# michaelwillett/GPU-ICP-SLAM

Measured on AMD Instinct MI355X. Metric: particle-scan evals/sec (1081 beams x N particles), full particleFilter step, KD path, higher is better.
Workload: dtype f32; 1 GPU; synthetic 1081-beam scans, 100000 particles/GPU, 100000-point KD map, full SLAM step (disperse+score+weights+ICP/SVD+map update+resample); particles_global=100000, parallelism=particles sharded x1, map replicated, kd_size_end=191383

## Files before the change

### gpu-icp-slam_amd/build.py

```python
import fcntl
import hashlib
import os
import shutil
import subprocess

HERE = os.path.dirname(os.path.abspath(__file__))
CSRC = os.path.join(HERE, "csrc")
OBJ = os.path.join(HERE, "build")
LIB = os.path.join(HERE, "libpfslam_hip.so")
INC = os.path.join("..", "..", "include", "pfslam.h")
UNITS = {
    "pfslam_hip.hip": ["pf_math.h", "kd_device.h", "kd_cells.hip.inc", "pfslam_stages.hip.inc", "pfslam_frame.hip.inc", "pfslam_register.hip.inc", "pfslam_register_batch.hip.inc", "pfslam_search.hip.inc", "pfslam_search_scan.hip.inc", "pfslam_search_cov.hip.inc", "pfslam_search_wide.hip.inc", "pfslam_search_best.hip.inc", INC],
    "kd_host.cpp": [INC],
}
FLAGS = ["--offload-arch=gfx950", "-O3", "-std=c++17", "-ffp-contract=off", "-fPIC",
         "-Wall", "-Wno-unused-function", "-Wno-unused-result"] + os.environ.get("PFSLAM_EXTRA_FLAGS", "").split()


def hipcc():
    for c in (os.environ.get("HIPCC"), "/opt/rocm/bin/hipcc", shutil.which("hipcc")):
        if c and os.path.exists(c):
            return c
    raise RuntimeError("hipcc not found: libpfslam_hip.so cannot be built (there is no CPU fallback)")


def _digest(files):
    h = hashlib.sha1(" ".join(FLAGS).encode())
    for f in files:
        with open(os.path.join(CSRC, f), "rb") as fh:
            h.update(f.encode() + b"\0" + fh.read())
    return h.hexdigest()


def _unit_digest(src, deps):
    return _digest([src] + deps)


def _read(path):
    try:
        with open(path) as fh:
            return fh.read().strip()
    except OSError:
        return ""


# ... 40 lines not shown
```

### gpu-icp-slam_amd/csrc/kd_cells.hip.inc

```

#define PF_CELL_SUB 2
#define PF_CELL_WIN (2560 * PF_CELL_SUB)
#define PF_CELL_LIST_CAP (1 << 19)
#define PF_CELL_POOL_CAP (1 << 22)
#define PF_CELL_MAXC 12
#define PF_CELL_RUN 32
#define PF_CELL_MAXR 14
#define PF_CELL_MARK_MAX 4096
#define PF_CELL_PENDING 0xFFFFFFFFu
#define PF_CELL_FALLBACK 0xFFFFFFFEu
enum { PF_CS_COUNT = 0, PF_CS_POOL, PF_CS_SNAP, PF_CS_PAD3, PF_CS_LIST_CAP, PF_CS_POOL_CAP, PF_CS_FLAGS, PF_CS_PAD, PF_CS_ROWS, PF_CS_N1, PF_CS_N2,
       PF_CS_NONE, PF_CS_CUR_FRESH, PF_CS_CUR_EXT, PF_CS_CUR_REUSED, PF_CS_CUR_CLAIMED, PF_CS_WORDS = 32,
       PF_CS_OX = 128, PF_CS_OY = 129, PF_CS_ALLOC = 256 };
#define PF_CF_LIST_FULL 1
#define PF_CF_POOL_FULL 2
#define PF_CF_NEED_ORIGIN 4
#define PF_CF_FAR 8
#define PF_CELL_DRIFT_MAX 120
#define PF_REC_WORDS 96
#define PF_REC_TERM 4
#define PF_REC_CAND 20
#define PF_REC_PAR 36
#define PF_REC_RC 52
#define PF_REC_POOL 76
// ... 783 lines not shown
#undef S_CY
#undef S_PP
#undef S_PC
#undef S_CT
#undef S_PI
#undef S_R
#undef S_RX
#undef S_RY
__device__ __forceinline__ float cell_dist2(const uint4 cd, float wx, float wy)
{
    typedef float f32x2 __attribute__((ext_vector_type(2)));
    const f32x2 nxy = {__uint_as_float(cd.x), __uint_as_float(cd.y)};
    const f32x2 pxy = {wx, wy};
    const f32x2 d = nxy - pxy;
    const f32x2 dd = d * d;
    return dd.x + dd.y;
}
__device__ __forceinline__ bool cell_visit(const uint4 cd, float wx, float wy, float &sBest)
{
    const float s = cell_dist2(cd, wx, wy);
    const float sGuard = sBest * PF_GUARD_K;
    bool take = s < sGuard;
    const bool inBand = (s < sBest) != take;
    if (__builtin_amdgcn_ballot_w64(inBand) != 0ull) {
        float sb = sBest;
        asm volatile("" : "+v"(sb));
        take = take | (inBand && pf::fsqrt(s) < pf::fsqrt(sb));
    }
    sBest = take ? s : sBest;
    return take;
}

#define PF_ROW_SLACK 4
template <bool CENSUS = false, int GUARD = 1>
__global__ __launch_bounds__(64) void k_score_kd_cells(const float *__restrict__ px, const float *__restrict__ py,
                                                       const float *__restrict__ pth, int n, const float *__restrict__ scan,
                                                       const pf::BeamParts *__restrict__ beams, int nb, int beams_per_chunk, pf::KdView tree,
                                                       CellGeom geo, const unsigned *__restrict__ tab, const uint4 *__restrict__ pool,
                                                       const int *__restrict__ cs, const int *__restrict__ order, int direct,
                                                       float *__restrict__ out, int out_mode, pf::KdCensus *__restrict__ census = nullptr,
                                                       unsigned long long *__restrict__ probe = nullptr, const double2 *__restrict__ tparts = nullptr)
{
    pf_stamp(probe);
    const int g = blockIdx.x, slot = g * 64 + threadIdx.x;
    const int j0 = blockIdx.y * beams_per_chunk;
    const int j1 = min(nb, j0 + beams_per_chunk);
    const bool real = slot < n;
    const int i = order ? order[min(slot, n - 1)] : min(slot, n - 1);
    const float x = px[i], y = py[i], th = pth[i];
    pf::AngleParts T;
    if (tparts) {
        const double2 tp = tparts[i];
        T.c = tp.x;
        T.s = tp.y;
        T.a = (double)th;
    } else T = pf::angle_parts(th);
    const int ox = cs[PF_CS_OX], oy = cs[PF_CS_OY];
    const float inv2x = 2.0f * geo.invx, inv2y = 2.0f * geo.invy;
    const pf::kd_rsrc_t tab_rsrc = pf::kd_rsrc(tab), pool_rsrc = pf::kd_rsrc(pool);
    float acc = 0.0f, wpend = 0.0f;
    pf::KdCensusLocal cl = {0, 0, 0, 0, 0, 0, 0, 0};
    auto stage_a = [&](int j, float &wx, float &wy, unsigned &e) -> bool {
        const float r = scan[j];
        if (!(fabsf(r) < PF_RANGE_NEVER)) return false;
        beam_end_point<GUARD>(beams, j, r, th, T, wx, wy);
        if (!(fabsf(wx) < PF_LIDAR_RANGE && fabsf(wy) < PF_LIDAR_RANGE)) return false;
        wx += x;
        wy += y;
        e = 0u;
        float gx, gy;
        int cx = sub_index_fast(wx, inv2x, gx), cy = sub_index_fast(wy, inv2y, gy);
        const float g = fminf(gx, gy);
        bool ok = g > 0.0f;
        if (__builtin_amdgcn_fcmpf(g, 0.0f, 2 ) != __builtin_amdgcn_ballot_w64(true)) {
            if (!ok && fabsf(wx) < 1e6f && fabsf(wy) < 1e6f) {
                cx = sub_index(wx, geo.resx, geo.invx);
                cy = sub_index(wy, geo.resy, geo.invy);
                float lox, loy, hi, cell_lo;
                sub_edges(cx, geo.resx, lox, hi, cell_lo);
// ... 83 lines not shown
#pragma unroll
                    for (int q = 0; q < 4; q++)
                        if (k0 + q < n1) {
                            const bool take = cell_visit(cd[q], wx, wy, sBest);
                            pk = take ? cd[q].z : pk;
                            pcoord = take ? __uint_as_float(cd[q].w) : pcoord;
                        }
                }
                b = (int)(pk & 0x3fffffffu);
                if (pk < 0xC0000000u && n2 != 0) {
                    float hd = (pk < 0x40000000u ? wx : wy) - pcoord;
                    hd = (int)pk < 0 ? 0.0f : hd;
                    const float h2 = hd * hd;
                    bool pass = h2 < sBest * PF_GUARD_K;
                    const bool inBand = (!pass && h2 * PF_GUARD_K <= sBest) || sBest < 1e-30f;
                    if (__builtin_amdgcn_ballot_w64(inBand) != 0ull) {
                        float sb = sBest;
                        asm volatile("" : "+v"(sb));
                        pass = inBand ? fabsf(hd) < pf::fsqrt(sb) : pass;
                    }
                    if (pass) b = resolve(wx, wy, sBest, b, off + n1, n2);
                }
            }
            acc += wpend;
            wpend = tree.w[b];
        }
        cok = nok; cwx = nwx; cwy = nwy; ce = ne;
    }
    acc += wpend;
    if (CENSUS) pf::census_flush(cl, census);
    if (real && out_mode == 0) out[(size_t)blockIdx.y * n + (direct ? i : slot)] = acc;
    if (real && out_mode == 3) ((short *)out)[(size_t)blockIdx.y * n + slot] = (short)(int)acc;
    if (out_mode == 4) ((short *)out)[((size_t)g * gridDim.y + blockIdx.y) * 64 + threadIdx.x] = real ? (short)(int)acc : (short)0;
}
```

### gpu-icp-slam_amd/csrc/pfslam_frame.hip.inc

```

#define PF_FRAME_RING 4
enum { PF_FS_BOUND = 0, PF_FS_WALKED = 4, PF_FS_TICKET = 8, PF_FS_ICP = 9, PF_FS_WORDS = 16 };
enum { PF_WC_WALLS = 0, PF_WC_NEW, PF_WC_FLAGS, PF_WC_SIZE, PF_WC_WORDS = 4 };

enum { PF_FL_REDUCED = 0, PF_FL_TREE, PF_FL_ORDER, PF_FL_ICP, PF_FL_SCAN, PF_FL_FTAIL, PF_FL_POSEG , PF_FL_WORDS = 8 };
__device__ __forceinline__ void flag_store(int *word, int ticket) { __hip_atomic_store(word, ticket, __ATOMIC_RELEASE, __HIP_MEMORY_SCOPE_AGENT); }
__device__ __forceinline__ bool flag_wait(const int *word, int ticket, int *err)
{
    const unsigned long long t0 = wall_clock64(), limit = g_gate_ticks;
    while (__hip_atomic_load(word, __ATOMIC_ACQUIRE, __HIP_MEMORY_SCOPE_AGENT) - ticket < 0) {
        __builtin_amdgcn_s_sleep(8);
        if (wall_clock64() - t0 > limit) {
            if (err) __hip_atomic_store(err, ticket, __ATOMIC_RELAXED, __HIP_MEMORY_SCOPE_SYSTEM);
            return false;
        }
    }
    return true;
}
__global__ void k_gate(const int *__restrict__ word, int ticket, int *__restrict__ err)
{
    if (threadIdx.x == 0) flag_wait(word, ticket, err);
}
__global__ void k_gate_signal(int *__restrict__ done_word, int done_ticket, const int *__restrict__ word, int ticket, int *__restrict__ err)
{
// ... 908 lines not shown
    CHK(dalloc(&h->cloud, 8));
    HIPCHK(hipMemsetAsync(h->cloud, 0, 32, h->stream));
    CHK(dalloc(&h->sigr, (size_t)PF_FRAME_RING * 80));
    HIPCHK(hipMemsetAsync(h->sigr, 0, (size_t)PF_FRAME_RING * 80 * 4, h->stream));
    CHK(dalloc(&h->order_ring, (size_t)PF_FRAME_RING * h->n));
    hipEvent_t *evs[] = {&h->ev_reduced, &h->ev_tree2, &h->ev_order, &h->ev_icp, &h->ev_ftail, &h->ev_shift, &h->ev_poseg,
                         &h->ev_marked_r[0], &h->ev_marked_r[1], &h->ev_marked_r[2], &h->ev_marked_r[3],
                         &h->ev_walked_r[0], &h->ev_walked_r[1], &h->ev_walked_r[2], &h->ev_walked_r[3],
                         &h->ev_tail[0], &h->ev_tail[1], &h->ev_tail[2]};
    for (hipEvent_t *e : evs) HIPCHK(pf_event_create(e, hipEventDisableTiming));
    return 0;
}
static int gates_decide(pfslam_handle *h, bool *use)
{
    if (h->gates && !h->gates_tested) {
        if (h->pipe_live) CHK(settle_staged(h));
        hipStream_t st[4] = {h->stream, h->aux, h->fstream, h->cstream};
        for (hipStream_t q : st) HIPCHK(hipStreamSynchronize(q));
        bool ok = false;
        CHK(gates_selftest(h, &ok));
        h->gates_ok = ok;
        h->gates_tested = true;
        if (!ok && getenv("PFSLAM_VERBOSE")) fprintf(stderr, "pfslam: streams share a hardware queue: the frame's cross-stream edges stay events\n");
    }
    const bool want = h->gates && h->gates_ok && g_live_handles.load() == 1;
    if (h->pipe_live && want != h->gates_live) CHK(settle_staged(h));
    h->gates_live = want;
    *use = want;
    return 0;
}

static void frame_free(pfslam_handle *h)
{
    void *bufs[] = {h->fs, h->wcounts, h->flags, h->order_tmp, h->tparts, h->wall_c2, h->wall_xy2, h->wall_leaf2, h->wall_new2, h->wall_runs, h->wall_keys_s, h->wall_c2s, h->fstats, h->cloud, h->sigr, h->order_ring, h->pgroup, h->probe};
    for (void *b : bufs)
        if (b) (void)hipFree(b);
    hipEvent_t evs[] = {h->ev_reduced, h->ev_tree2, h->ev_order, h->ev_icp, h->ev_ftail, h->ev_shift, h->ev_poseg,
                        h->ev_marked_r[0], h->ev_marked_r[1], h->ev_marked_r[2], h->ev_marked_r[3],
                        h->ev_walked_r[0], h->ev_walked_r[1], h->ev_walked_r[2], h->ev_walked_r[3], h->ev_tail[0], h->ev_tail[1], h->ev_tail[2]};
    for (hipEvent_t e : evs)
        if (e) (void)hipEventDestroy(e);
    if (h->gate_err) (void)hipHostFree(h->gate_err);
}

static int join_all(pfslam_handle *h)
{
    if (!h->pipe_live || h->serial) return 0;
    hipStream_t tails[3] = {h->aux, h->fstream, h->cstream};
    for (int k = 0; k < 3; k++) {
        HIPCHK(hipEventRecord(h->ev_tail[k], tails[k]));
        HIPCHK(hipStreamWaitEvent(h->stream, h->ev_tail[k], 0));
    }
    return 0;
}

static bool frame_v2_ok(pfslam_handle *h, int *chunks_out, int *bpc_out)
{
    if (h->timing >= 2 || h->kd_size <= 0 || !h->integral_w || h->nb > 4096) return false;
    if (!org_use_cells(h, nullptr, true)) return false;
    const int chunks = score_chunks(h);
    const int bpc = (h->nb + chunks - 1) / chunks;
    const int used = (h->nb + bpc - 1) / bpc;
    if (used < 2 || !((float)bpc * h->w_absmax <= 32767.0f)) return false;
    if ((h->gn + PF_SCAN_TILE - 1) / PF_SCAN_TILE > 4096) return false;
    *chunks_out = used;
    *bpc_out = bpc;
    return true;
}

static int probe_slot_ptr(pfslam_handle *h, int id, unsigned long long **out)
{
    *out = (h->probe && h->probe_frames > 0) ? h->probe + (size_t)(h->cur_seq % h->probe_frames) * PF_PROBE_SLOTS + id : nullptr;
    return 0;
}
#define PB(id) (h->probe ? h->probe + (size_t)(seq % h->probe_frames) * PF_PROBE_SLOTS + (id) : (unsigned long long *)nullptr)

struct FvCtx {
    hipStream_t P, C, F, K;
    int seq, s4, s2, lag, groups, world;
    bool gates, serial, sync_cells, sharded, multi, ftail_gate;
    CellGeom geo;
    pf::KdView tv;
    long long *stats, *stats_next;
    float *sig, *sig_next, *icp_dbg;
    int *order, *fl;
    HostHeader *hdr;
    PoseSrc psrc;
};
static FvCtx fv_ctx(pfslam_handle *h)
{
    FvCtx c;
    const auto &fv = h->fv;
    c.serial = fv.serial;
    c.sync_cells = fv.sync_cells;
    c.sharded = fv.sharded;
// ... 50 lines not shown
    HIPCHK(hipEventRecord(h->ev_marked_r[s4], K));
    if (!c.sync_cells && h->pipe_live) FV_EDGE_WAIT(K, PF_FL_TREE, h->ev_tree2, 1);
    if (c.sync_cells) {
        h->cells_passes++;
        hipLaunchKernelGGL(k_cells_update<true>, dim3(PF_CELLS_GRID), dim3(64), 0, K, c.tv, c.geo, h->cell_tab, (const int *)h->cell_list, h->cell_state, h->cell_pool,
                           h->cell_rec, h->cells_gen, (const int *)nullptr, 0, 0, 0, CellPass{nullptr, nullptr, nullptr, nullptr, 0}, PB(PB_WALK));
        hipLaunchKernelGGL(k_fs_walked, dim3(1), dim3(64), 0, K, h->fs, (const int *)h->cell_state);
    } else {
        hipLaunchKernelGGL(k_cells_update<false>, dim3(PF_CELLS_WALK_GRID), dim3(64), 0, K, c.tv, c.geo, h->cell_tab, (const int *)h->cell_list, h->cell_state,
                           h->cell_pool, h->cell_rec, h->cells_gen, (const int *)nullptr, 0, 0, 0,
                           CellPass{h->fs + PF_FS_WALKED + ((seq - 1) & 3), h->fs + PF_FS_WALKED + s4, nullptr, h->fs + PF_FS_BOUND + s4, 0}, PB(PB_WALK));
    }
    HIPCHK(hipGetLastError());
    HIPCHK(hipEventRecord(h->ev_walked_r[s4], K));
    return 0;
}

static int frame_v2_begin(pfslam_handle *h, int frame, const float *scan_host, int used, int bpc, bool sharded)
{
    CHK(frame_alloc(h));
    if (!h->cell_tab) CHK(cells_alloc(h));
    const int groups = (h->n + 63) / 64;
    if (!h->group_box) CHK(dalloc(&h->group_box, (size_t)groups));
    if (!h->group_parts) CHK(dalloc(&h->group_parts, (size_t)groups));
    {
        const size_t need = (size_t)groups * used * 64;
        if (need > h->pgroup_elems) {
            if (h->pgroup) HIPCHK(hipFree(h->pgroup));
            h->pgroup = nullptr;
            CHK(dalloc(&h->pgroup, need));
            h->pgroup_elems = need;
        }
    }
    bool gates = false;
    CHK(gates_decide(h, &gates));
    const bool sync_cells = h->cells_wipe_pending;
    const bool serial = h->serial != 0 || sync_cells;
    if (!h->pipe_live) {
        CHK(settle(h));
        HIPCHK(hipStreamSynchronize(h->stream));
        HIPCHK(hipStreamSynchronize(h->aux));
        HIPCHK(hipStreamSynchronize(h->cstream));
        HIPCHK(hipStreamSynchronize(h->istream));
        hipLaunchKernelGGL(k_fs_init, dim3(1), dim3(64), 0, h->stream, h->fs, (const int *)h->kd_state,
                           sync_cells ? (const int *)nullptr : (const int *)h->cell_state, h->fstats);
        HIPCHK(hipMemsetAsync(h->sigr, 0, (size_t)PF_FRAME_RING * 80 * 4, h->stream));
        HIPCHK(hipGetLastError());
        h->cloud_valid = false;
        h->shift_pending = false;
        h->icp_forked = h->map_forked = h->walk_pending = h->cells_snap = h->tree_event = h->mark_on_aux = false;
        HIPCHK(hipStreamSynchronize(h->stream));
    } else if (serial) {
        CHK(join_all(h));
    }
    const int seq = ++h->seq;
    h->cur_seq = seq;
    h->cur_frame = frame;
    h->fv.used = used;
    h->fv.bpc = bpc;
    h->fv.frame = frame;
    h->fv.sync_cells = sync_cells;
    h->fv.serial = serial;
    h->fv.sharded = sharded;
    h->fv.gates = gates;
    h->fv.ftail_gate = gates && !serial;
    h->x_frame = h->x; h->y_frame = h->y; h->th_frame = h->th;
    const FvCtx c = fv_ctx(h);
    hipStream_t P = c.P, F = c.F;
    int *fl = c.fl;
    const bool ftail_gate = c.ftail_gate;

    if (sync_cells) CHK(cells_wipe(h));
    {
        const int bits = h->n <= 400000 ? 6 : PF_CELL_BITS_MAX, ncell = 1 << (3 * bits);
        int *hist = h->cells, *cursor = h->cells + ncell, *tile_tot = h->cells + 2 * ncell;
        float *cloud_in = h->cloud + 4 * (c.s2 ^ 1), *cloud_out = h->cloud + 4 * c.s2;
        {
            float *hs = h->h_scan + (size_t)(seq % PF_HDR_SLOTS) * h->nb;
            h->scan = h->scan_base + (size_t)(seq % PF_HDR_SLOTS) * h->nb;
            memcpy(hs, scan_host, (size_t)h->nb * 4);
            scan_reach_of(h, hs);
            if (h->probe && h->probe_frames > 0)
                HIPCHK(hipMemsetAsync(h->probe + (size_t)(seq % h->probe_frames) * PF_PROBE_SLOTS, 0, (size_t)PF_PROBE_SLOTS * 8, P));
            HIPCHK(hipMemcpyAsync(h->scan, hs, (size_t)h->nb * 4, hipMemcpyHostToDevice, P));
            if (gates && !serial) hipLaunchKernelGGL(k_signal, dim3(1), dim3(64), 0, P, fl + PF_FL_SCAN, seq);
        }
        const float reach = h->scan_reach;
        h->tparts_cur = nullptr;
        if (!h->cloud_valid) {
            hipLaunchKernelGGL(k_cloud_seed, dim3(1), dim3(256), 0, P, (const float *)h->x, (const float *)h->y, (const float *)h->th, h->n, reach, cloud_in, c.sig);
            h->cloud_valid = true;
        }
        hipLaunchKernelGGL(k_motion_count, dim3((h->n + 255) / 256), dim3(256), 0, P, h->x, h->y, h->th, h->w, (const float *)h->wm, h->n, frame, h->goff,
                           reach, bits, h->mkey, hist, h->cell_state, c.geo, (const float *)cloud_in, cloud_out, c.sig, c.sig_next, PB(PB_MOTION), (double2 *)nullptr, h->trig);
        hipLaunchKernelGGL(k_cell_scan, dim3(ncell / 1024), dim3(256), 0, P, hist, cursor, tile_tot);
        hipLaunchKernelGGL(k_cell_scatter, dim3((h->n + 255) / 256), dim3(256), 0, P, h->mkey, h->n, cursor, tile_tot, ncell / 1024, c.order);
        if (h->stable_order) {
            if (!h->order_tmp) CHK(dalloc(&h->order_tmp, (size_t)h->n));
            hipLaunchKernelGGL(k_order_stable, dim3((h->n + 255) / 256), dim3(256), 0, P, (const int *)c.order, (const unsigned *)h->mkey, h->n, h->order_tmp);
            HIPCHK(hipMemcpyAsync(c.order, h->order_tmp, (size_t)h->n * 4, hipMemcpyDeviceToDevice, P));
        }
        HIPCHK(hipGetLastError());
        if (h->pipe_live && !serial) {
            if (ftail_gate) hipLaunchKernelGGL(k_gate, dim3(1), dim3(64), 0, P, (const int *)(fl + PF_FL_FTAIL), seq - 1, h->gate_err_dev);
            else if (h->ftail_recorded) HIPCHK(hipStreamWaitEvent(P, h->ev_ftail, 0));
        }
        if (gates) hipLaunchKernelGGL(k_signal, dim3(1), dim3(64), 0, P, fl + PF_FL_ORDER, seq);
        else HIPCHK(hipEventRecord(h->ev_order, P));
        h->theta_bound += 0.1f;
    }
    if (sync_cells || h->mark_early != 0) CHK(fv_cells_passes(h, c));
    {
        if (ftail_gate) {
            hipLaunchKernelGGL(k_gate_signal, dim3(1), dim3(64), 0, F, fl + PF_FL_FTAIL, seq - 1, (const int *)(fl + PF_FL_SCAN), seq, h->gate_err_dev);
            HIPCHK(hipGetLastError());
        } else FV_EDGE_WAIT(F, PF_FL_ORDER, h->ev_order, 0);
// ... 2 lines not shown
        const dim3 gi((h->nb + 1023) / 1024);
        if (h->planar)
            hipLaunchKernelGGL(k_icp_fused<true>, gi, dim3(1024), 0, F, (const float *)h->scan, h->nb, (const float *)h->pose, c.tv, (float4 *)h->icp_tar,
                               (float4 *)h->icp_cor, c.icp_dbg, h->fs + PF_FS_ICP, PB(PB_ICP), gates ? fl : (int *)nullptr, seq, h->trig);
        else
            hipLaunchKernelGGL(k_icp_fused<false>, gi, dim3(1024), 0, F, (const float *)h->scan, h->nb, (const float *)h->pose, c.tv, (float4 *)h->icp_tar,
                               (float4 *)h->icp_cor, c.icp_dbg, h->fs + PF_FS_ICP, PB(PB_ICP), gates ? fl : (int *)nullptr, seq, h->trig);
        HIPCHK(hipGetLastError());
        if (!gates) HIPCHK(hipEventRecord(h->ev_icp, F));
    }
    return 0;
}

static int frame_v2_score(pfslam_handle *h)
{
    const FvCtx c = fv_ctx(h);
    const int seq = c.seq, used = h->fv.used, bpc = h->fv.bpc, groups = c.groups;
    hipStream_t P = c.P, C = c.C;
    if (c.multi) {
        hipLaunchKernelGGL(k_theta_gmax, dim3(std::min(256, (h->world * h->stride + 255) / 256)), dim3(256), 0, P, (const float *)h->gpose, h->world, h->stride, h->gtheta,
                           seq, c.gates ? c.fl + PF_FL_POSEG : (int *)nullptr);
        HIPCHK(hipGetLastError());
        if (!c.gates) HIPCHK(hipEventRecord(h->ev_poseg, P));
    }
    FV_EDGE_WAIT(C, PF_FL_ORDER, h->ev_order, 0);
    hipEvent_t t_a = nullptr, t_b = nullptr;
    if (h->timing) {
        CHK(timer_event(h, &t_a));
        CHK(timer_event(h, &t_b));
        HIPCHK(hipEventRecord(t_a, C));
    }
    const bool guard = !(h->theta_bound < 0.5f * PF_SUM_THETA_MAX) || (c.multi && !h->theta_global_known);
    const dim3 grid64(groups, used);
#define PF_CELLS_ARGS grid64, dim3(64), 0, C, h->x_frame, h->y_frame, h->th_frame, h->n, h->scan, (const pf::BeamParts *)h->beam_angle, h->nb, bpc, c.tv, c.geo, \
                      (const unsigned *)h->cell_tab, (const uint4 *)h->cell_pool, (const int *)h->cell_state, (const int *)c.order, 0
    if (h->trig) hipLaunchKernelGGL((k_score_kd_cells<false, PF_TRIG_DEVLIB>), PF_CELLS_ARGS, (float *)h->pgroup, 4, (pf::KdCensus *)nullptr, PB(PB_SCORE), (const double2 *)nullptr);
    else if (guard) hipLaunchKernelGGL((k_score_kd_cells<false, true>), PF_CELLS_ARGS, (float *)h->pgroup, 4, (pf::KdCensus *)nullptr, PB(PB_SCORE), (const double2 *)nullptr);
    else hipLaunchKernelGGL((k_score_kd_cells<false, false>), PF_CELLS_ARGS, (float *)h->pgroup, 4, (pf::KdCensus *)nullptr, PB(PB_SCORE), (const double2 *)nullptr);
    HIPCHK(hipGetLastError());
    if (t_a) {
        HIPCHK(hipEventRecord(t_b, C));
        h->ev_pending.push_back(pfslam_handle::TimedSpan{t_a, t_b, PF_T_SCORE});
    }
    if (h->census_log && h->census_n < PF_CENSUS_LOG) {
        if (h->trig) hipLaunchKernelGGL((k_score_kd_cells<true, PF_TRIG_DEVLIB>), PF_CELLS_ARGS, (float *)h->pgroup, 2, h->census_log + h->census_n++, (unsigned long long *)nullptr);
        else hipLaunchKernelGGL((k_score_kd_cells<true, true>), PF_CELLS_ARGS, (float *)h->pgroup, 2, h->census_log + h->census_n++, (unsigned long long *)nullptr);
        HIPCHK(hipGetLastError());
    }
#undef PF_CELLS_ARGS
    if (!c.gates) HIPCHK(hipStreamWaitEvent(C, h->ev_icp, 0));
    if (used >= 256)
        hipLaunchKernelGGL((k_reduce_groups<4>), dim3(groups), dim3(256), 0, C, (const short *)h->pgroup, h->n, groups, used, (const int *)c.order, h->fit, c.stats,
                           PB(PB_REDUCE), h->goff);
    else {
        hipLaunchKernelGGL((k_reduce_groups<1>), dim3(std::min((groups + 3) / 4, PF_REDUCE_WGS)), dim3(256), 0, C, (const short *)h->pgroup, h->n, groups, used,
                           (const int *)c.order, h->fit, c.stats, PB(PB_REDUCE), h->goff);
    }
    HIPCHK(hipGetLastError());
    return 0;
}

static int frame_v2_chain(pfslam_handle *h)
{
    const FvCtx c = fv_ctx(h);
    const int seq = c.seq, s4 = c.s4, lag = c.lag;
    hipStream_t P = c.P, C = c.C;
    const bool gates = c.gates, serial = c.serial, sync_cells = c.sync_cells;
    int *fl = c.fl;
    {
        if (!gates) {
            HIPCHK(hipEventRecord(h->ev_reduced, C));
            if (c.multi) HIPCHK(hipStreamWaitEvent(C, h->ev_poseg, 0));
        }
        if (!sync_cells && h->mark_early == 0) CHK(fv_cells_passes(h, c));
        const int sort_n = (h->nb + 63) / 64 * 64;
        const size_t lds = (size_t)sort_n * 9 * sizeof(uint32_t);
        if (!h->walls_attr_set) {
            HIPCHK(hipFuncSetAttribute((const void *)k_walls<0>, hipFuncAttributeMaxDynamicSharedMemorySize, (int)lds));
            HIPCHK(hipFuncSetAttribute((const void *)k_walls<3>, hipFuncAttributeMaxDynamicSharedMemorySize, (int)lds));
// ... 148 lines not shown
```

### gpu-icp-slam_amd/csrc/pfslam_hip.hip

```cpp
#include "../../include/pfslam.h"
#include "kd_device.h"
#include "pf_math.h"

#include <hip/hip_runtime.h>

#include <algorithm>
#include <atomic>
#include <deque>
#include <thread>
#include <cmath>
#include <cstdio>
#include <chrono>
#include <cstring>
#include <string>
#include <vector>

#define PF_LIDAR_RANGE 20.0f
#define PF_RANGE_NEVER 28.4f
#define PF_FREE_WEIGHT (-1)
#define PF_OCCUPIED_WEIGHT 4
#define PF_EFFECTIVE_PARTICLES .7
#define PF_CLAMP_VAL 113.0f
#define PF_SUM_EXACT 16777216.0f
#define PF_SVD_EPSILON 0.00001f
#define PF_SUM_TILE 4096
#define PF_SCAN_TILE 1024
#define PF_SCAN_CHUNK 16
enum { PF_T_SCORE = 0, PF_T_MOTION, PF_T_MEASURE, PF_T_MAP, PF_T_RESAMPLE, PF_T_PLAN, PF_TIMER_SLOTS };
#define PF_CENSUS_LOG 1024
#define PF_KD_MAX_NODES ((1 << 27) - 1)


__device__ unsigned long long g_gate_ticks = 100000000ull;
#define PF_GATE_TICKS_SHARDED 6000000000ull

// ... 92 lines not shown
    unsigned long long *wide_state = nullptr;
    size_t wide_field_cap = 0, wide_ends_cap = 0, wide_nin_cap = 0, wide_nodes_cap = 0, wide_lb_cap = 0;
    int wide_frontier = 0;
    unsigned long long *best_tab = nullptr, *best_list = nullptr, *best_state = nullptr;
    size_t best_tab_cap = 0, best_list_cap = 0;
    float *scan_in = nullptr;
    float2 *scan_pts = nullptr;
    unsigned long long *scan_state = nullptr;
    float *cov_part = nullptr;
    size_t cov_part_cap = 0;
    unsigned long long *cov_state = nullptr;
    float *est_part = nullptr;
    int8_t *grid = nullptr;
    int32_t *fit_i = nullptr;
    std::vector<int8_t> h_grid;
    struct TopoNode { float x, y, dist; };
    std::vector<TopoNode> topo_nodes{TopoNode{0.0f, 0.0f, 0.0f}};
    std::vector<std::vector<unsigned>> topo_edges{std::vector<unsigned>()};
    unsigned topo_idx = 0;
    int *d_count = nullptr;
    int topo_in_step = 0;
    hipStream_t topo_stream = nullptr;
    std::vector<int32_t> frame_closures;
    HostHeader *h_hdr = nullptr, *hdr_dev = nullptr;
    float *h_scan = nullptr;
    struct Frame { int seq, frame, kind; bool boxes = false; bool v2 = false; bool gtheta = false; };
    std::deque<Frame> in_flight;
    int seq = 0;
    int cur_seq = 0, cur_frame = 0;
    int shard_stage = 0;
    bool shard_v2 = false;
    bool shard_call = false;
    bool theta_global_known = true;
    struct FrameV2 { int used = 0, bpc = 0, frame = 0; bool sync_cells = false, serial = false, sharded = false, gates = false, ftail_gate = false; } fv;
    bool gates_tested = false;
    bool gates_ok = false;
    bool gates_live = false;
    hipEvent_t ev_poseg = nullptr;
    int lag = 1;
    float scan_reach = 8.0f;
    std::vector<pfslam_particle> h_particles;
    std::vector<float> h_tmp;
    int32_t trace[8] = {0};
    hipEvent_t ev0 = nullptr, ev1 = nullptr;
    hipStream_t aux = nullptr;
    hipEvent_t ev_fork = nullptr, ev_join = nullptr;
    hipEvent_t ev_mapfork = nullptr, ev_map = nullptr;
    bool map_forked = false;
    bool scan_front_done = false;
    bool header_packed = false;
    bool lds_attr_set = false;
    bool mirror_stale = false;
    int mirror_n = 0;
    bool icp_forked = false;
    bool icp_delta_ready = false;
    bool masks_cleared = false;
    bool stats_clean = false;
    int timing = 0;
    struct TimedSpan { hipEvent_t a, b; int slot; bool keep_b = false; };
    std::vector<hipEvent_t> ev_pool;
    std::vector<TimedSpan> ev_pending;
    hipEvent_t phase_ev = nullptr;
    double timer_ms[PF_TIMER_SLOTS] = {0};
    long timer_count[PF_TIMER_SLOTS] = {0};
    pf::KdCensus *d_census = nullptr;
    pf::KdCensus *census_store = nullptr, *census_log = nullptr;
    int census_n = 0;
// ... 27 lines not shown
    hipEvent_t ev_boxes = nullptr;
    hipEvent_t ev_marked = nullptr;
    bool mark_on_aux = false;
    hipStream_t istream = nullptr;
    hipEvent_t ev_tree = nullptr;
    void *pin_tree = nullptr;
    bool tree_event = false;
    hipStream_t cstream = nullptr;
    hipEvent_t ev_walked = nullptr;
    bool walk_pending = false;
    bool update_unsnapped = false;
    bool cells_snap = false;
    pf::BeamParts *beam_angle = nullptr;
    int resampler = 0;
    int trig = 0;
    int serial = 0;
    bool pipe_live = false;
    bool cloud_valid = false;
    int publish_lag = 2;
    int *fs = nullptr;
    int *wcounts = nullptr;
    float2 *wall_xy2 = nullptr;
    int *wall_leaf2 = nullptr, *wall_new2 = nullptr;
    int *wall_c2 = nullptr;
    uint32_t *wall_runs = nullptr, *wall_keys_s = nullptr;
    double2 *tparts = nullptr, *tparts_cur = nullptr;
    int *wall_c2s = nullptr;
    long long *fstats = nullptr;
    float *cloud = nullptr;
    float *sigr = nullptr;
    int *order_ring = nullptr;
    short *pgroup = nullptr;
    size_t pgroup_elems = 0;
    hipStream_t fstream = nullptr;
    hipEvent_t ev_reduced = nullptr, ev_tree2 = nullptr, ev_order = nullptr, ev_icp = nullptr, ev_ftail = nullptr, ev_shift = nullptr;
    hipEvent_t ev_marked_r[4] = {nullptr, nullptr, nullptr, nullptr}, ev_walked_r[4] = {nullptr, nullptr, nullptr, nullptr};
    hipEvent_t ev_tail[3] = {nullptr, nullptr, nullptr};
    int fault = 0;
    int stable_order = 0;
    int *order_tmp = nullptr;
    int mark_early = 1;
    int gates = 1;
    bool ftail_recorded = false;
    int *flags = nullptr;
    int *gate_err = nullptr, *gate_err_dev = nullptr;
    const float *x_frame = nullptr, *y_frame = nullptr, *th_frame = nullptr;
    bool shift_pending = false;
    bool balance_done = false;
    bool walls_attr_set = false;
    unsigned long long *probe = nullptr;
    int probe_frames = 0;
};
#define PF_PROBE_SLOTS 32
enum { PB_ICP = 0, PB_MOTION, PB_SCATTER, PB_BOX, PB_MARK, PB_WALK, PB_SCORE, PB_REDUCE, PB_WALLS, PB_UPDATE, PB_WEIGHTS, PB_APPLY, PB_GATHER, PB_RAYS, PB_COUNT,
       PB_LISTS, PB_FREE, PB_WALLW, PB_REDUCE_LAST, PB_WALLS_KEYS, PB_WALLS_SORTED, PB_WALLS_TRAV, PB_WALLS_END, PB_WALLS_REP, PB_ICP_SOLVE, PB_ICP_END, PB_UPDATE_END, PB_REDUCE_END, PB_END };
static const char *const pb_names[PB_END] = {"K icp", "P motion+cells", "P scatter", "K boxes", "K mark", "K walk", "C scan-match", "C reduce", "C walls+insert",
                                             "C cells update", "P weights", "P scan apply", "P sample+gather", "F rays", "F count", "F lists", "F free pass", "F wall weights",
                                             "C reduce: last wg", "C walls: keys", "C walls: sorted", "C walls: traversed", "C walls: end", "C walls: traversal launch", "K icp: solve", "K icp: end", "C cells update: last wg ends", "C reduce: last wg ends"};
static_assert(PB_END <= PF_PROBE_SLOTS, "probe slots");


__global__ __launch_bounds__(256) void k_motion(float *__restrict__ x, float *__restrict__ y,
                                                float *__restrict__ th, float *__restrict__ w,
                                                const float *__restrict__ wm, int n, int frame, int goff, int trig = 0)
{
    int i = blockIdx.x * 256 + threadIdx.x;
    if (i >= n) return;
    w[i] = wm[i];
    uint32_t e2 = pf::engine_seed(frame, goff + i, 0);
    const float sx = 0.015, sy = 0.015, st = .01;
    float nx = pf::normal(e2, 0.0f, sx, trig != 0);
    float ny = pf::normal(e2, 0.0f, sy, trig != 0);
    float nt = pf::normal(e2, 0.0f, st, trig != 0);
    x[i] += nx;
    y[i] += ny;
    th[i] += nt;
}

__global__ void k_beam_angles(pf::BeamParts *__restrict__ beams, int nb)
{
    const int j = blockIdx.x * blockDim.x + threadIdx.x;
    if (j >= nb) return;
    const float angle = pf::lidar_angle(j);
    const pf::AngleParts p = pf::angle_parts(angle);
    beams[j] = pf::BeamParts{p.c, p.s, p.a, angle, 0.0f};
}
template <int GUARD = 1>
__device__ __forceinline__ void beam_end_point(const pf::BeamParts *__restrict__ beams, int j, float range, float theta, const pf::AngleParts &T,
                                               float &x, float &y)
{
    const pf::BeamParts bp = beams[j];
// ... 1072 lines not shown
}
extern "C" int pfslam_shift_particles(pfslam_handle *h, const float delta[3])
{
    if (!h || !delta) return fail("pfslam_shift_particles: bad argument");
    HIPCHK(hipSetDevice(h->cfg.device));
    CHK(join_map(h));
    if (h->pipe_live && !h->serial) {
        HIPCHK(hipEventRecord(h->ev_tail[0], h->aux));
        HIPCHK(hipStreamWaitEvent(h->stream, h->ev_tail[0], 0));
        if (!h->ftail_recorded) {
            HIPCHK(hipEventRecord(h->ev_ftail, h->fstream));
            h->ftail_recorded = true;
        }
        HIPCHK(hipStreamWaitEvent(h->stream, h->ev_ftail, 0));
    }
    const float ad = delta[2] == delta[2] ? fabsf(delta[2]) : INFINITY;
    h->theta_shift += ad;
    h->theta_bound += ad;
    h->theta_shift_seq = h->seq;
    hipLaunchKernelGGL(k_shift, dim3((h->n + 255) / 256), dim3(256), 0, h->stream, h->x, h->y, h->th, h->n, delta[0], delta[1], delta[2], h->pose,
                       h->cloud_valid ? h->cloud : (float *)nullptr);
    HIPCHK(hipGetLastError());
    if (h->pipe_live) {
        HIPCHK(hipEventRecord(h->ev_shift, h->stream));
        h->shift_pending = true;
    }
    return 0;
}

static int score_chunks(const pfslam_handle *h)
{
    const int groups = (h->n + 63) / 64;
    const int target = std::max(24576, std::min(65536, groups * 160));
    int chunks = (target + groups - 1) / groups;
    chunks = std::max(1, std::min(chunks, h->nb));
    if (!h->integral_w) chunks = 1;
    return chunks;
}

#define PF_CELLS_WALK_GRID 32
#define PF_CELLS_GRID 512
#define PF_CELLS_RECUT_EVERY 16
#define PF_CELLS_BOX_MAX 24.0f
struct CellArgs { unsigned *tab; int *list, *cs; uint4 *pool; int *rec; };
__global__ void k_cells_reset(int *cs, int list_cap, int pool_cap)
{
    if (threadIdx.x < PF_CS_WORDS)
        cs[threadIdx.x] = threadIdx.x == PF_CS_FLAGS ? PF_CF_NEED_ORIGIN : threadIdx.x == PF_CS_LIST_CAP ? list_cap : threadIdx.x == PF_CS_POOL_CAP ? pool_cap : 0;
}
static int cells_wipe(pfslam_handle *h)
{
    HIPCHK(hipMemsetAsync(h->cell_tab, 0, (size_t)PF_CELL_WIN * PF_CELL_WIN * 4, h->stream));
    static const int list_cap = getenv("PFSLAM_CELL_LIST_CAP") ? std::min(std::max(atoi(getenv("PFSLAM_CELL_LIST_CAP")), 64), PF_CELL_LIST_CAP) : PF_CELL_LIST_CAP;
    static const int pool_cap = getenv("PFSLAM_CELL_POOL_CAP") ? std::min(std::max(atoi(getenv("PFSLAM_CELL_POOL_CAP")), 64), PF_CELL_POOL_CAP) : PF_CELL_POOL_CAP;
    hipLaunchKernelGGL(k_cells_reset, dim3(1), dim3(64), 0, h->stream, h->cell_state, list_cap, pool_cap);
    HIPCHK(hipGetLastError());
    h->cells_wipe_pending = false;
    h->cells_wipe_seq = h->seq;
    h->cells_wipes++;
    h->cells_gen++;
    h->cells_passes = 0;
    return 0;
}
static int launch_cells_update(pfslam_handle *h, hipStream_t st)
{
    if (!h->cell_tab || h->cells_wipe_pending) return 0;
    const CellGeom geo{h->cfg.map_res_x, h->cfg.map_res_y, 1.0f / h->cfg.map_res_x, 1.0f / h->cfg.map_res_y};
    const int recut = h->cells_passes > 0 && h->cells_passes % PF_CELLS_RECUT_EVERY == 0 ? 1 : 0;
// ... 472 lines not shown
extern "C" int pfslam_debug_check_cells(pfslam_handle *h, long long out[16])
{
    if (!h || !out) return fail("pfslam_debug_check_cells: bad argument");
    for (int k = 0; k < 16; k++) out[k] = 0;
    if (!h->cell_tab || !h->cells_valid || h->cells_wipe_pending) return 0;
    HIPCHK(hipSetDevice(h->cfg.device));
    CHK(settle(h));
    unsigned long long *d = nullptr;
    CHK(dalloc(&d, 16));
    HIPCHK(hipMemsetAsync(d, 0, 128, h->stream));
    hipLaunchKernelGGL(k_cells_check, dim3(2048), dim3(256), 0, h->stream, kd_view(h), (const unsigned *)h->cell_tab, (const int *)h->cell_list,
                       (const int *)h->cell_state, (const uint4 *)h->cell_pool, (const int *)h->cell_rec, h->cells_gen, d);
    HIPCHK(hipGetLastError());
    int cs[PF_CS_WORDS];
    HIPCHK(hipMemcpyAsync(out, d, 128, hipMemcpyDeviceToHost, h->stream));
    HIPCHK(hipMemcpyAsync(cs, h->cell_state, sizeof(cs), hipMemcpyDeviceToHost, h->stream));
    HIPCHK(hipStreamSynchronize(h->stream));
    HIPCHK(hipFree(d));
    if (!(cs[PF_CS_FLAGS] & (PF_CF_LIST_FULL | PF_CF_POOL_FULL)))
        out[15] = (out[4] != cs[PF_CS_ROWS]) + (out[6] != cs[PF_CS_NONE]) + (out[5] != out[1] + out[2]);
    return 0;
}

extern "C" int pfslam_set_probe(pfslam_handle *h, int frames)
{
    if (!h || frames < 0 || frames > 4096) return fail("pfslam_set_probe: 0 .. 4096 frames");
    HIPCHK(hipSetDevice(h->cfg.device));
    CHK(settle(h));
    HIPCHK(hipStreamSynchronize(h->stream));
    if (h->probe) HIPCHK(hipFree(h->probe));
    h->probe = nullptr;
    h->probe_frames = 0;
    if (frames > 0) {
        CHK(dalloc(&h->probe, (size_t)frames * PF_PROBE_SLOTS));
        HIPCHK(hipMemset(h->probe, 0, (size_t)frames * PF_PROBE_SLOTS * 8));
        h->probe_frames = frames;
    }
    return 0;
}
extern "C" int pfslam_get_probe(pfslam_handle *h, unsigned long long *out, int cap_frames, int *n_frames, int *last_ticket)
{
    if (!h || !n_frames || (cap_frames > 0 && !out)) return fail("pfslam_get_probe: bad argument");
    *n_frames = 0;
    if (last_ticket) *last_ticket = h->seq;
    if (!h->probe) return 0;
    HIPCHK(hipSetDevice(h->cfg.device));
    CHK(settle(h));
    HIPCHK(hipStreamSynchronize(h->stream));
    const int n = std::min(std::min(cap_frames, h->probe_frames), h->seq);
    std::vector<unsigned long long> all((size_t)h->probe_frames * PF_PROBE_SLOTS);
    HIPCHK(hipMemcpy(all.data(), h->probe, all.size() * 8, hipMemcpyDeviceToHost));
    for (int k = 0; k < n; k++) {
        const int ticket = h->seq - n + 1 + k;
        memcpy(out + (size_t)k * PF_PROBE_SLOTS, &all[(size_t)(ticket % h->probe_frames) * PF_PROBE_SLOTS], PF_PROBE_SLOTS * 8);
    }
    *n_frames = n;
    return 0;
}
extern "C" int pfslam_frame_mode(pfslam_handle *h, int out[4])
{
    if (!h || !out) return fail("pfslam_frame_mode: bad argument");
    out[0] = h->pipe_live ? 1 : 0;
    out[1] = h->pipe_live ? (h->gates_live ? 1 : 0) : h->gates;
    out[2] = h->serial;
    out[3] = h->publish_lag;
    return 0;
}
extern "C" const char *pfslam_probe_name(int slot) { return slot >= 0 && slot < PB_END ? pb_names[slot] : ""; }
extern "C" int pfslam_set_trig(pfslam_handle *h, int devlib)
{
    if (!h || devlib < 0 || devlib > 1) return fail("pfslam_set_trig: 0 (specification) or 1 (device library)");
    HIPCHK(hipSetDevice(h->cfg.device));
    CHK(settle(h));
    h->trig = devlib;
    return 0;
}
extern "C" int pfslam_set_resampler(pfslam_handle *h, int mode)
{
    if (!h || mode < 0 || mode > 2) return fail("pfslam_set_resampler: 0 (reference seeding), 1 (per-particle seeds) or 2 (systematic)");
    HIPCHK(hipSetDevice(h->cfg.device));
    CHK(settle(h));
    h->resampler = mode;
    return 0;
}
extern "C" int pfslam_set_serial(pfslam_handle *h, int serial)
{
    if (!h) return fail("null handle");
// ... 161 lines not shown
```

Measured before the change: 173.9 million particle-scan evals/s.

## Taper scan-match beam chunk sizes to shrink the score kernel tail

Adds a host-side score plan that splits the beams into non-uniform chunks: full-size body chunks followed by progressively smaller tail chunks. The chunk boundaries are uploaded once to the device, and the cells scoring kernel reads per-chunk start/end indices. The aim is to cut tail idle time when the last waves of the grid run with fewer active blocks. In exchange the grid gets a few more chunks, the partial-sum buffer grows, and there is a one-time stream sync to upload the plan. The change also adds probe instrumentation that records when the last scoring wave starts and ends.

After: 179.4 million particle-scan evals/s, median of 6. 3.1% higher.

```diff
diff --git a/gpu-icp-slam_amd/build.py b/gpu-icp-slam_amd/build.py
--- a/gpu-icp-slam_amd/build.py
+++ b/gpu-icp-slam_amd/build.py
@@ -10,7 +10,7 @@
 LIB = os.path.join(HERE, "libpfslam_hip.so")
 INC = os.path.join("..", "..", "include", "pfslam.h")
 UNITS = {
-    "pfslam_hip.hip": ["pf_math.h", "kd_device.h", "kd_cells.hip.inc", "pfslam_stages.hip.inc", "pfslam_frame.hip.inc", "pfslam_register.hip.inc", "pfslam_register_batch.hip.inc", "pfslam_search.hip.inc", "pfslam_search_scan.hip.inc", "pfslam_search_cov.hip.inc", "pfslam_search_wide.hip.inc", "pfslam_search_best.hip.inc", INC],
+    "pfslam_hip.hip": ["pf_math.h", "kd_device.h", "score_plan.h", "kd_cells.hip.inc", "pfslam_stages.hip.inc", "pfslam_frame.hip.inc", "pfslam_register.hip.inc", "pfslam_register_batch.hip.inc", "pfslam_search.hip.inc", "pfslam_search_scan.hip.inc", "pfslam_search_cov.hip.inc", "pfslam_search_wide.hip.inc", "pfslam_search_best.hip.inc", INC],
     "kd_host.cpp": [INC],
 }
 FLAGS = ["--offload-arch=gfx950", "-O3", "-std=c++17", "-ffp-contract=off", "-fPIC",
diff --git a/gpu-icp-slam_amd/csrc/kd_cells.hip.inc b/gpu-icp-slam_amd/csrc/kd_cells.hip.inc
--- a/gpu-icp-slam_amd/csrc/kd_cells.hip.inc
+++ b/gpu-icp-slam_amd/csrc/kd_cells.hip.inc
@@ -839,19 +839,21 @@
 }
 
 #define PF_ROW_SLACK 4
-template <bool CENSUS = false, int GUARD = 1>
+template <bool CENSUS = false, int GUARD = 1, bool ENDS = false>
 __global__ __launch_bounds__(64) void k_score_kd_cells(const float *__restrict__ px, const float *__restrict__ py,
                                                        const float *__restrict__ pth, int n, const float *__restrict__ scan,
                                                        const pf::BeamParts *__restrict__ beams, int nb, int beams_per_chunk, pf::KdView tree,
                                                        CellGeom geo, const unsigned *__restrict__ tab, const uint4 *__restrict__ pool,
                                                        const int *__restrict__ cs, const int *__restrict__ order, int direct,
                                                        float *__restrict__ out, int out_mode, pf::KdCensus *__restrict__ census = nullptr,
-                                                       unsigned long long *__restrict__ probe = nullptr, const double2 *__restrict__ tparts = nullptr)
+                                                       unsigned long long *__restrict__ probe = nullptr, const double2 *__restrict__ tparts = nullptr,
+                                                       const int *__restrict__ starts = nullptr, unsigned long long *__restrict__ probe_ends = nullptr)
 {
     pf_stamp(probe);
+    if (probe && blockIdx.x == gridDim.x - 1 && blockIdx.y == gridDim.y - 1 && threadIdx.x == 0) probe[PB_SCORE_LAST - PB_SCORE] = wall_clock64();
     const int g = blockIdx.x, slot = g * 64 + threadIdx.x;
-    const int j0 = blockIdx.y * beams_per_chunk;
-    const int j1 = min(nb, j0 + beams_per_chunk);
+    const int j0 = starts ? starts[blockIdx.y] : blockIdx.y * beams_per_chunk;
+    const int j1 = starts ? starts[blockIdx.y + 1] : min(nb, j0 + beams_per_chunk);
     const bool real = slot < n;
     const int i = order ? order[min(slot, n - 1)] : min(slot, n - 1);
     const float x = px[i], y = py[i], th = pth[i];
@@ -1001,4 +1003,5 @@
     if (real && out_mode == 0) out[(size_t)blockIdx.y * n + (direct ? i : slot)] = acc;
     if (real && out_mode == 3) ((short *)out)[(size_t)blockIdx.y * n + slot] = (short)(int)acc;
     if (out_mode == 4) ((short *)out)[((size_t)g * gridDim.y + blockIdx.y) * 64 + threadIdx.x] = real ? (short)(int)acc : (short)0;
-}
+    if (ENDS && probe_ends && threadIdx.x == 0) atomicMax(probe_ends + (blockIdx.x & (PF_PROBE_ENDS - 1)) * PF_PROBE_END_STRIDE, (unsigned long long)wall_clock64());
+}
diff --git a/gpu-icp-slam_amd/csrc/pfslam_frame.hip.inc b/gpu-icp-slam_amd/csrc/pfslam_frame.hip.inc
--- a/gpu-icp-slam_amd/csrc/pfslam_frame.hip.inc
+++ b/gpu-icp-slam_amd/csrc/pfslam_frame.hip.inc
@@ -964,7 +964,7 @@
 
 static void frame_free(pfslam_handle *h)
 {
-    void *bufs[] = {h->fs, h->wcounts, h->flags, h->order_tmp, h->tparts, h->wall_c2, h->wall_xy2, h->wall_leaf2, h->wall_new2, h->wall_runs, h->wall_keys_s, h->wall_c2s, h->fstats, h->cloud, h->sigr, h->order_ring, h->pgroup, h->probe};
+    void *bufs[] = {h->fs, h->wcounts, h->flags, h->order_tmp, h->tparts, h->wall_c2, h->wall_xy2, h->wall_leaf2, h->wall_new2, h->wall_runs, h->wall_keys_s, h->wall_c2s, h->fstats, h->cloud, h->sigr, h->order_ring, h->pgroup, h->probe, h->plan_starts};
     for (void *b : bufs)
         if (b) (void)hipFree(b);
     hipEvent_t evs[] = {h->ev_reduced, h->ev_tree2, h->ev_order, h->ev_icp, h->ev_ftail, h->ev_shift, h->ev_poseg,
@@ -990,9 +990,14 @@
 {
     if (h->timing >= 2 || h->kd_size <= 0 || !h->integral_w || h->nb > 4096) return false;
     if (!org_use_cells(h, nullptr, true)) return false;
-    const int chunks = score_chunks(h);
-    const int bpc = (h->nb + chunks - 1) / chunks;
-    const int used = (h->nb + bpc - 1) / bpc;
+    if (h->plan_n != h->n || h->plan_nb != h->nb || h->plan_w != h->w_absmax) {
+        h->chunk_plan = pf::score_plan(h->n, h->nb, h->w_absmax, h->integral_w != 0);
+        h->plan_n = h->n;
+        h->plan_nb = h->nb;
+        h->plan_w = h->w_absmax;
+        h->plan_uploaded = false;
+    }
+    const int used = h->chunk_plan.used, bpc = h->chunk_plan.bpc;
     if (used < 2 || !((float)bpc * h->w_absmax <= 32767.0f)) return false;
     if ((h->gn + PF_SCAN_TILE - 1) / PF_SCAN_TILE > 4096) return false;
     *chunks_out = used;
@@ -1109,6 +1114,18 @@
             h->pgroup_elems = need;
         }
     }
+    if (h->chunk_plan.tapered && !h->plan_uploaded) {
+        for (hipStream_t st : {h->stream, h->aux, h->cstream, h->istream}) HIPCHK(hipStreamSynchronize(st));
+        if ((int)h->chunk_plan.starts.size() > h->plan_starts_cap) {
+            if (h->plan_starts) HIPCHK(hipFree(h->plan_starts));
+            h->plan_starts = nullptr;
+            h->plan_starts_cap = 0;
+            CHK(dalloc(&h->plan_starts, h->chunk_plan.starts.size()));
+            h->plan_starts_cap = (int)h->chunk_plan.starts.size();
+        }
+        HIPCHK(hipMemcpy(h->plan_starts, h->chunk_plan.starts.data(), h->chunk_plan.starts.size() * 4, hipMemcpyHostToDevice));
+        h->plan_uploaded = true;
+    }
     bool gates = false;
     CHK(gates_decide(h, &gates));
     const bool sync_cells = h->cells_wipe_pending;
@@ -1135,6 +1152,7 @@
     h->cur_frame = frame;
     h->fv.used = used;
     h->fv.bpc = bpc;
+    h->fv.starts = h->chunk_plan.tapered ? h->plan_starts : nullptr;
     h->fv.frame = frame;
     h->fv.sync_cells = sync_cells;
     h->fv.serial = serial;
@@ -1157,8 +1175,11 @@
             h->scan = h->scan_base + (size_t)(seq % PF_HDR_SLOTS) * h->nb;
             memcpy(hs, scan_host, (size_t)h->nb * 4);
             scan_reach_of(h, hs);
-            if (h->probe && h->probe_frames > 0)
+            if (h->probe && h->probe_frames > 0) {
                 HIPCHK(hipMemsetAsync(h->probe + (size_t)(seq % h->probe_frames) * PF_PROBE_SLOTS, 0, (size_t)PF_PROBE_SLOTS * 8, P));
+                HIPCHK(hipMemsetAsync(h->probe + (size_t)h->probe_frames * PF_PROBE_SLOTS + (size_t)(seq % h->probe_frames) * PF_PROBE_ENDS * PF_PROBE_END_STRIDE, 0,
+                                      (size_t)PF_PROBE_ENDS * PF_PROBE_END_STRIDE * 8, P));
+            }
             HIPCHK(hipMemcpyAsync(h->scan, hs, (size_t)h->nb * 4, hipMemcpyHostToDevice, P));
             if (gates && !serial) hipLaunchKernelGGL(k_signal, dim3(1), dim3(64), 0, P, fl + PF_FL_SCAN, seq);
         }
@@ -1227,19 +1248,27 @@
     }
     const bool guard = !(h->theta_bound < 0.5f * PF_SUM_THETA_MAX) || (c.multi && !h->theta_global_known);
     const dim3 grid64(groups, used);
+    const int *starts = h->fv.starts;
+    unsigned long long *ends = h->probe ? h->probe + (size_t)h->probe_frames * PF_PROBE_SLOTS + (size_t)(seq % h->probe_frames) * PF_PROBE_ENDS * PF_PROBE_END_STRIDE : nullptr;
 #define PF_CELLS_ARGS grid64, dim3(64), 0, C, h->x_frame, h->y_frame, h->th_frame, h->n, h->scan, (const pf::BeamParts *)h->beam_angle, h->nb, bpc, c.tv, c.geo, \
                       (const unsigned *)h->cell_tab, (const uint4 *)h->cell_pool, (const int *)h->cell_state, (const int *)c.order, 0
-    if (h->trig) hipLaunchKernelGGL((k_score_kd_cells<false, PF_TRIG_DEVLIB>), PF_CELLS_ARGS, (float *)h->pgroup, 4, (pf::KdCensus *)nullptr, PB(PB_SCORE), (const double2 *)nullptr);
-    else if (guard) hipLaunchKernelGGL((k_score_kd_cells<false, true>), PF_CELLS_ARGS, (float *)h->pgroup, 4, (pf::KdCensus *)nullptr, PB(PB_SCORE), (const double2 *)nullptr);
-    else hipLaunchKernelGGL((k_score_kd_cells<false, false>), PF_CELLS_ARGS, (float *)h->pgroup, 4, (pf::KdCensus *)nullptr, PB(PB_SCORE), (const double2 *)nullptr);
+#define PF_CELLS_TAIL (float *)h->pgroup, 4, (pf::KdCensus *)nullptr, PB(PB_SCORE), (const double2 *)nullptr, starts, ends
+    if (ends) {
+        if (h->trig) hipLaunchKernelGGL((k_score_kd_cells<false, PF_TRIG_DEVLIB, true>), PF_CELLS_ARGS, PF_CELLS_TAIL);
+        else if (guard) hipLaunchKernelGGL((k_score_kd_cells<false, true, true>), PF_CELLS_ARGS, PF_CELLS_TAIL);
+        else hipLaunchKernelGGL((k_score_kd_cells<false, false, true>), PF_CELLS_ARGS, PF_CELLS_TAIL);
+    } else if (h->trig) hipLaunchKernelGGL((k_score_kd_cells<false, PF_TRIG_DEVLIB>), PF_CELLS_ARGS, PF_CELLS_TAIL);
+    else if (guard) hipLaunchKernelGGL((k_score_kd_cells<false, true>), PF_CELLS_ARGS, PF_CELLS_TAIL);
+    else hipLaunchKernelGGL((k_score_kd_cells<false, false>), PF_CELLS_ARGS, PF_CELLS_TAIL);
+#undef PF_CELLS_TAIL
     HIPCHK(hipGetLastError());
     if (t_a) {
         HIPCHK(hipEventRecord(t_b, C));
         h->ev_pending.push_back(pfslam_handle::TimedSpan{t_a, t_b, PF_T_SCORE});
     }
     if (h->census_log && h->census_n < PF_CENSUS_LOG) {
-        if (h->trig) hipLaunchKernelGGL((k_score_kd_cells<true, PF_TRIG_DEVLIB>), PF_CELLS_ARGS, (float *)h->pgroup, 2, h->census_log + h->census_n++, (unsigned long long *)nullptr);
-        else hipLaunchKernelGGL((k_score_kd_cells<true, true>), PF_CELLS_ARGS, (float *)h->pgroup, 2, h->census_log + h->census_n++, (unsigned long long *)nullptr);
+        if (h->trig) hipLaunchKernelGGL((k_score_kd_cells<true, PF_TRIG_DEVLIB>), PF_CELLS_ARGS, (float *)h->pgroup, 2, h->census_log + h->census_n++, (unsigned long long *)nullptr, (const double2 *)nullptr, starts);
+        else hipLaunchKernelGGL((k_score_kd_cells<true, true>), PF_CELLS_ARGS, (float *)h->pgroup, 2, h->census_log + h->census_n++, (unsigned long long *)nullptr, (const double2 *)nullptr, starts);
         HIPCHK(hipGetLastError());
     }
 #undef PF_CELLS_ARGS
diff --git a/gpu-icp-slam_amd/csrc/pfslam_hip.hip b/gpu-icp-slam_amd/csrc/pfslam_hip.hip
--- a/gpu-icp-slam_amd/csrc/pfslam_hip.hip
+++ b/gpu-icp-slam_amd/csrc/pfslam_hip.hip
@@ -1,6 +1,7 @@
 #include "../../include/pfslam.h"
 #include "kd_device.h"
 #include "pf_math.h"
+#include "score_plan.h"
 
 #include <hip/hip_runtime.h>
 
@@ -159,7 +160,7 @@
     bool shard_v2 = false;
     bool shard_call = false;
     bool theta_global_known = true;
-    struct FrameV2 { int used = 0, bpc = 0, frame = 0; bool sync_cells = false, serial = false, sharded = false, gates = false, ftail_gate = false; } fv;
+    struct FrameV2 { int used = 0, bpc = 0, frame = 0; const int *starts = nullptr; bool sync_cells = false, serial = false, sharded = false, gates = false, ftail_gate = false; } fv;
     bool gates_tested = false;
     bool gates_ok = false;
     bool gates_live = false;
@@ -253,6 +254,12 @@
     int *order_ring = nullptr;
     short *pgroup = nullptr;
     size_t pgroup_elems = 0;
+    pf::ScorePlan chunk_plan;
+    int plan_n = -1, plan_nb = -1;
+    float plan_w = -1.0f;
+    int *plan_starts = nullptr;
+    int plan_starts_cap = 0;
+    bool plan_uploaded = false;
     hipStream_t fstream = nullptr;
     hipEvent_t ev_reduced = nullptr, ev_tree2 = nullptr, ev_order = nullptr, ev_icp = nullptr, ev_ftail = nullptr, ev_shift = nullptr;
     hipEvent_t ev_marked_r[4] = {nullptr, nullptr, nullptr, nullptr}, ev_walked_r[4] = {nullptr, nullptr, nullptr, nullptr};
@@ -273,11 +280,15 @@
     int probe_frames = 0;
 };
 #define PF_PROBE_SLOTS 32
+#define PF_PROBE_ENDS 64
+#define PF_PROBE_END_STRIDE 16
+#define PF_PROBE_ROW (PF_PROBE_SLOTS + PF_PROBE_ENDS * PF_PROBE_END_STRIDE)
 enum { PB_ICP = 0, PB_MOTION, PB_SCATTER, PB_BOX, PB_MARK, PB_WALK, PB_SCORE, PB_REDUCE, PB_WALLS, PB_UPDATE, PB_WEIGHTS, PB_APPLY, PB_GATHER, PB_RAYS, PB_COUNT,
-       PB_LISTS, PB_FREE, PB_WALLW, PB_REDUCE_LAST, PB_WALLS_KEYS, PB_WALLS_SORTED, PB_WALLS_TRAV, PB_WALLS_END, PB_WALLS_REP, PB_ICP_SOLVE, PB_ICP_END, PB_UPDATE_END, PB_REDUCE_END, PB_END };
+       PB_LISTS, PB_FREE, PB_WALLW, PB_REDUCE_LAST, PB_WALLS_KEYS, PB_WALLS_SORTED, PB_WALLS_TRAV, PB_WALLS_END, PB_WALLS_REP, PB_ICP_SOLVE, PB_ICP_END, PB_UPDATE_END, PB_REDUCE_END, PB_SCORE_LAST, PB_SCORE_END, PB_END };
 static const char *const pb_names[PB_END] = {"K icp", "P motion+cells", "P scatter", "K boxes", "K mark", "K walk", "C scan-match", "C reduce", "C walls+insert",
                                              "C cells update", "P weights", "P scan apply", "P sample+gather", "F rays", "F count", "F lists", "F free pass", "F wall weights",
-                                             "C reduce: last wg", "C walls: keys", "C walls: sorted", "C walls: traversed", "C walls: end", "C walls: traversal launch", "K icp: solve", "K icp: end", "C cells update: last wg ends", "C reduce: last wg ends"};
+                                             "C reduce: last wg", "C walls: keys", "C walls: sorted", "C walls: traversed", "C walls: end", "C walls: traversal launch", "K icp: solve", "K icp: end", "C cells update: last wg ends", "C reduce: last wg ends",
+                                             "C scan-match: last wave starts", "C scan-match: last wave ends"};
 static_assert(PB_END <= PF_PROBE_SLOTS, "probe slots");
 
 
@@ -1416,8 +1427,7 @@
 {
     const int groups = (h->n + 63) / 64;
     const int target = std::max(24576, std::min(65536, groups * 160));
-    int chunks = (target + groups - 1) / groups;
-    chunks = std::max(1, std::min(chunks, h->nb));
+    int chunks = pf::score_plan_chunks_for(target, groups, h->nb);
     if (!h->integral_w) chunks = 1;
     return chunks;
 }
@@ -1956,8 +1966,8 @@
     h->probe = nullptr;
     h->probe_frames = 0;
     if (frames > 0) {
-        CHK(dalloc(&h->probe, (size_t)frames * PF_PROBE_SLOTS));
-        HIPCHK(hipMemset(h->probe, 0, (size_t)frames * PF_PROBE_SLOTS * 8));
+        CHK(dalloc(&h->probe, (size_t)frames * PF_PROBE_ROW));
+        HIPCHK(hipMemset(h->probe, 0, (size_t)frames * PF_PROBE_ROW * 8));
         h->probe_frames = frames;
     }
     return 0;
@@ -1972,11 +1982,15 @@
     CHK(settle(h));
     HIPCHK(hipStreamSynchronize(h->stream));
     const int n = std::min(std::min(cap_frames, h->probe_frames), h->seq);
-    std::vector<unsigned long long> all((size_t)h->probe_frames * PF_PROBE_SLOTS);
+    std::vector<unsigned long long> all((size_t)h->probe_frames * PF_PROBE_ROW);
     HIPCHK(hipMemcpy(all.data(), h->probe, all.size() * 8, hipMemcpyDeviceToHost));
     for (int k = 0; k < n; k++) {
-        const int ticket = h->seq - n + 1 + k;
-        memcpy(out + (size_t)k * PF_PROBE_SLOTS, &all[(size_t)(ticket % h->probe_frames) * PF_PROBE_SLOTS], PF_PROBE_SLOTS * 8);
+        const int ticket = h->seq - n + 1 + k, row = ticket % h->probe_frames;
+        memcpy(out + (size_t)k * PF_PROBE_SLOTS, &all[(size_t)row * PF_PROBE_SLOTS], PF_PROBE_SLOTS * 8);
+        const unsigned long long *ends = &all[(size_t)h->probe_frames * PF_PROBE_SLOTS + (size_t)row * PF_PROBE_ENDS * PF_PROBE_END_STRIDE];
+        unsigned long long last = 0;
+        for (int e = 0; e < PF_PROBE_ENDS; e++) last = std::max(last, ends[(size_t)e * PF_PROBE_END_STRIDE]);
+        out[(size_t)k * PF_PROBE_SLOTS + PB_SCORE_END] = last;
     }
     *n_frames = n;
     return 0;
diff --git a/gpu-icp-slam_amd/csrc/score_plan.h b/gpu-icp-slam_amd/csrc/score_plan.h
--- /dev/null
+++ b/gpu-icp-slam_amd/csrc/score_plan.h
@@ -0,0 +1,97 @@
+#pragma once
+
+#include <algorithm>
+#include <vector>
+
+#ifndef PF_TAPER_SLOTS
+#define PF_TAPER_SLOTS 16384
+#endif
+#ifndef PF_TAPER_DIV
+#define PF_TAPER_DIV 6
+#endif
+#define PF_TAPER_MIN_BPC 8
+#define PF_P16_MAX 32767.0f
+
+namespace pf {
+
+struct ScorePlan {
+    int chunks = 1;
+    int bpc = 0, used = 0;
+    bool tapered = false;
+    bool p16_ok = false;
+    std::vector<int> starts;
+};
+
+inline int score_plan_target(int n)
+{
+    const int groups = (n + 63) / 64;
+    return std::max(24576, std::min(65536, groups * 160));
+}
+inline int score_plan_chunks_for(int target, int groups, int nb)
+{
+    if (groups < 1 || nb < 1) return 1;
+    const int chunks = (target + groups - 1) / groups;
+    return std::max(1, std::min(chunks, nb));
+}
+inline int score_plan_chunks(int n, int nb, bool integral_w)
+{
+    return integral_w ? score_plan_chunks_for(score_plan_target(n), (n + 63) / 64, nb) : 1;
+}
+
+inline ScorePlan score_plan(int n, int nb, float w_absmax, bool integral_w, int taper_slots = PF_TAPER_SLOTS, int taper_div = PF_TAPER_DIV)
+{
+    ScorePlan p;
+    const int groups = (n + 63) / 64;
+    if (n < 1 || nb < 1) return p;
+    const int chunks = score_plan_chunks(n, nb, integral_w);
+    p.chunks = chunks;
+    p.bpc = (nb + chunks - 1) / chunks;
+    p.used = (nb + p.bpc - 1) / p.bpc;
+    auto uniform = [&]() {
+        p.tapered = false;
+        p.starts.resize((size_t)p.used + 1);
+        for (int k = 0; k <= p.used; k++) p.starts[k] = (int)std::min<long long>(nb, (long long)k * p.bpc);
+        p.p16_ok = integral_w && p.used >= 2 && (float)p.bpc * w_absmax <= PF_P16_MAX;
+    };
+    uniform();
+    if (!integral_w || p.bpc < PF_TAPER_MIN_BPC) return p;
+    int body = p.bpc;
+    if ((float)body * w_absmax > PF_P16_MAX) body = (int)std::min((float)body, PF_P16_MAX / w_absmax);
+    if (body < 1) return p;
+    while (body > 1 && (float)body * w_absmax > PF_P16_MAX) body--;
+    const int S = std::max(2, body / std::max(1, taper_div));
+    int T = taper_slots > 0 && body >= PF_TAPER_MIN_BPC ? std::max(4, taper_slots / groups) : 0;
+    T = std::min(T, (nb / body) / 2);
+    if (T < 2) T = 0;
+    if (T == 0 && body == p.bpc) return p;
+    std::vector<int> w;
+    long long W = 0;
+    for (int i = 1; i <= T; i++) {
+        const int t = body - ((body - S) * i + T / 2) / T;
+        w.push_back(t);
+        W += t;
+    }
+    const int U = std::max((int)((nb - W + body - 1) / body), chunks - T);
+    W += (long long)U * body;
+    const int R = U + T;
+    if (U < 1 || R > nb) return p;
+    std::vector<int> size((size_t)R);
+    long long acc = 0, prev = 0;
+    for (int k = 0; k < R; k++) {
+        acc += k < U ? body : w[(size_t)(k - U)];
+        const long long cut = (acc * nb + W / 2) / W;
+        size[(size_t)k] = (int)(cut - prev);
+        prev = cut;
+    }
+    std::sort(size.begin(), size.end(), [](int a, int b) { return a > b; });
+    if (size.back() < 1 || size.front() > body || prev != nb) return p;
+    p.bpc = size.front();
+    p.used = R;
+    p.tapered = true;
+    p.starts.assign((size_t)R + 1, 0);
+    for (int k = 0; k < R; k++) p.starts[(size_t)k + 1] = p.starts[(size_t)k] + size[(size_t)k];
+    p.p16_ok = R >= 2 && (float)p.bpc * w_absmax <= PF_P16_MAX;
+    return p;
+}
+
+}
```
